# sony/DiffRoll

Measured on AMD Instinct MI355X. Metric: piano-roll frames/sec (200-step sample), higher is better.
Workload: dtype f32

## Files before the change

diffroll_amd/_cabi.py:

```python
from __future__ import annotations

import ctypes as C
import os

_HERE = os.path.dirname(os.path.abspath(__file__))
LIB_PATH = os.environ.get("DR_LIB") or os.path.join(_HERE, "lib", "libdiffroll_amd.so")

DR_ABI_VERSION = 11
DR_OK, DR_EINVAL, DR_ESTATE, DR_EHIP, DR_ENOMEM, DR_ENAME, DR_ETIMEOUT = 0, -1, -2, -3, -4, -5, -6

SAMPLERS = {
    "ddpm_x0": 0,
    "cfdg_ddpm_x0": 1,
    "generation_ddpm_x0": 2,
    "inpainting_ddpm_x0": 3,
    "ddim_x0": 4,
    "cfdg_ddim_x0": 5,
    "ddpm": 6,
    "ddim": 7,
    "ddim2ddpm": 8,
}
COND_SPEC, COND_UNCOND = 0, 1
PRECISIONS = {"f32": 0, "bf16x3": 1, "bf16": 2, "f16": 4}
NORM_MODES = {"imagewise": 0, "framewise": 1}

EXPORTS = [
    "dr_abi_version", "dr_create", "dr_destroy", "dr_last_error", "dr_set_param", "dr_set_tables", "dr_set_frontend_tables",
    "dr_commit", "dr_frontend", "dr_forward", "dr_forward_steps", "dr_step", "dr_sample", "dr_sample_checked", "dr_finish",
    "dr_pending_timeout", "dr_launch_state", "dr_note_runs", "dr_frame_counts", "dr_q_sample", "dr_extract_x0",
    "dr_set_spec_norm", "dr_set_precision", "dr_set_option",
    "dr_comm_unique_id", "dr_comm_create", "dr_comm_destroy", "dr_comm_info", "dr_comm_last_error", "dr_gather",
]
DEBUG_EXPORTS = [
    "dr_debug_stft_power", "dr_debug_bounds", "dr_debug_tenants", "dr_debug_kfd_root", "dr_debug_set_option", "dr_debug_ticks",
    "dr_stack_status", "dr_cold_times", "dr_profile_enable", "dr_profile_read", "dr_profile_read_ex",
    "dr_bench_layer", "dr_bench_pointwise", "dr_debug_launch_counts", "dr_debug_threshold", "dr_debug_rescale", "dr_debug_project",
    "dr_debug_momentum",
]
PUBLIC_OPTIONS = ("blocked_accumulation", "fused_rearm", "fused_stack", "fused_tail", "window_overlap", "window_break", "window_blend", "sampling_steps", "draws", "draw_stride",
                  "guidance_t_min", "guidance_t_max", "solver_order", "start_step", "start_noise", "solver_noise", "x0_clip", "x0_threshold", "cfg_rescale",
                  "cfg_project", "cfg_norm", "cfg_momentum", "guidance_stride")
MODES = {0: "none", 1: "per_phase", 2: "fused_stack", 3: "fused_stack+tail"}


class DrConfig(C.Structure):
    _fields_ = [
        ("abi_version", C.c_int32), ("device", C.c_int32),
        ("residual_channels", C.c_int32), ("residual_layers", C.c_int32),
        ("kernel_size", C.c_int32), ("dilation_base", C.c_int32), ("dilation_bound", C.c_int32),
        ("n_mels", C.c_int32), ("timesteps", C.c_int32), ("sample_rate", C.c_int32),
        ("n_fft", C.c_int32), ("hop_length", C.c_int32),
        ("f_min", C.c_float), ("f_max", C.c_float), ("beta_start", C.c_float), ("beta_end", C.c_float),
# ... 89 lines not shown
    lib.dr_profile_read.restype = C.c_int
    lib.dr_profile_read.argtypes = [vp, C.POINTER(C.c_int64), C.POINTER(C.c_double), C.c_int]
    lib.dr_profile_read_ex.restype = C.c_int
    lib.dr_profile_read_ex.argtypes = [vp, C.POINTER(C.c_int64), C.POINTER(C.c_double), C.POINTER(C.c_double),
                                       C.c_char_p, C.c_size_t, C.c_int]
    lib.dr_set_option.restype = C.c_int
    lib.dr_set_option.argtypes = [vp, C.c_char_p, C.c_int]
    lib.dr_stack_status.restype = C.c_int
    lib.dr_stack_status.argtypes = [vp, C.POINTER(C.c_int32), C.POINTER(C.c_int64), C.POINTER(C.c_int64), C.c_int]
    lib.dr_bench_layer.restype = C.c_int
    lib.dr_bench_layer.argtypes = [vp, C.c_int, C.c_int, C.c_int, C.c_int, C.c_int, vp]
    lib.dr_bench_pointwise.restype = C.c_int
    lib.dr_bench_pointwise.argtypes = [vp, C.c_int, C.c_int, C.c_int, vp]
    lib.dr_debug_ticks.restype = C.c_int
    lib.dr_debug_ticks.argtypes = [vp, C.POINTER(C.c_int64), C.POINTER(C.c_int64)]
    lib.dr_debug_launch_counts.restype = C.c_int
    lib.dr_debug_launch_counts.argtypes = [vp, C.POINTER(C.c_int64)]
    lib.dr_debug_threshold.restype = C.c_int
    lib.dr_debug_threshold.argtypes = [vp, vp, vp, C.c_int, C.c_int, C.c_float, vp, vp]
    lib.dr_debug_rescale.restype = C.c_int
    lib.dr_debug_rescale.argtypes = [vp, vp, vp, C.c_int, C.c_int, C.c_float, vp, vp]
    lib.dr_debug_project.restype = C.c_int
    lib.dr_debug_project.argtypes = [vp, vp, vp, C.c_int, C.c_int, C.c_float, vp, vp]
    lib.dr_debug_momentum.restype = C.c_int
    lib.dr_debug_momentum.argtypes = [vp, vp, vp, vp, vp, C.c_int, C.c_int, C.c_float, vp, vp]
    lib.dr_comm_unique_id.restype = C.c_int
    lib.dr_comm_unique_id.argtypes = [C.c_char_p]
    lib.dr_comm_create.restype = C.c_int
    lib.dr_comm_create.argtypes = [C.POINTER(vp), C.c_char_p, C.c_int, C.c_int, C.c_int]
    lib.dr_comm_destroy.restype = None
# ... 12 lines not shown
```

diffroll_amd/build.py:

```python
from __future__ import annotations

import os
import shutil
import subprocess
import sys

HERE = os.path.dirname(os.path.abspath(__file__))
CSRC = os.path.join(HERE, "csrc")
LIBDIR = os.path.join(HERE, "lib")
LIB = os.path.join(LIBDIR, "libdiffroll_amd.so")
SOURCES = ["gemm.hip", "stack.hip", "tail.hip", "update.hip", "threshold.hip", "rescale.hip", "project.hip", "momentum.hip", "stride.hip", "frontend.hip", "pack.hip", "plan.hip", "abi.hip", "debug_abi.hip", "comm.hip"]
HEADERS = [os.path.join(CSRC, h) for h in ("kernels.h", "chain_tables.h", "device_common.h", "gemm_body.h", "persistent.h", "update_quad.h", "threshold_quad.h", "rescale_quad.h", "project_quad.h", "momentum_quad.h", "stride_quad.h", "group_sums.h", "engine_state.h", "device_buffer.h", "captured_chain.h", "fused_mode.h", "launch_plan.h", "tenants.h", "f16_round.h")] + \
          [os.path.join(os.path.dirname(HERE), "include", h) for h in ("diffroll_amd.h", "diffroll_amd_debug.h")]
FLAGS = ["--offload-arch=gfx950", "-O3", "-std=c++17", "-fPIC", "-Wall", "-Wno-unused-function"]


def _hipcc() -> str:
    for cand in (os.environ.get("HIPCC"), shutil.which("hipcc"), "/opt/rocm/bin/hipcc"):
        if cand and os.path.exists(cand):
            return cand
    raise RuntimeError("hipcc not found (need ROCm with gfx950 support)")


def _stale(target: str, deps) -> bool:
    if not os.path.exists(target):
        return True
    t = os.path.getmtime(target)
# ... 77 lines not shown
```

diffroll_amd/csrc/abi.hip:

```cpp
#include "engine_state.h"
#include "tenants.h"

#include <algorithm>
#include <condition_variable>
#include <mutex>

namespace drh {

thread_local std::string g_create_error;
void release_stager(int dev);
std::atomic<int> g_engines[MAX_DEVICES];

struct FusedSlot {
    std::mutex mu;
    std::condition_variable cv;
    dr_engine* owner = nullptr;
    bool claimed = false;
    hipEvent_t done = nullptr;
};
FusedSlot g_slots[MAX_DEVICES];

bool claim_fused_slot(dr_engine* e, hipStream_t st) {
    FusedSlot& s = g_slots[e->cfg.device];
    std::unique_lock<std::mutex> lk(s.mu);
// ... 406 lines not shown
    if (n == "fused_stack_warm") { put(e, e->opt_stack_warm, value); return DR_OK; }
#ifdef DR_FAULT_HOOK
    if (n == "stack_fault_test") { put(e, e->opt_stack_fault, value); return DR_OK; }
#endif
    if (n == "stack_ticks") { put(e, e->stack_dbg_on, value); return DR_OK; }
    if (n.compare(0, 5, "tune.") == 0) {
        Tuning& t = tuning();
        const std::string f = n.substr(5);
        if (f == "ksplit_blocks") {
            if (put(e, t.ksplit_blocks, value)) tuning_epoch().fetch_add(1);
            return DR_OK;
        }
        std::atomic<int>* field = f == "pack_threads" ? &t.pack_threads : f == "tile" ? &t.tile : f == "pw" ? &t.pw : f == "pw_nw" ? &t.pw_nw
                   : f == "pwk" ? &t.pwk : f == "ksplit_max" ? &t.ksplit_max : f == "one_ks" ? &t.one_ks : f == "stack3" ? &t.stack3
                   : f == "stack_fl" ? &t.stack_fl : f == "tail_t4" ? &t.tail_t4 : f == "xcd_n" ? &t.xcd_n : f == "xcd_model" ? &t.xcd_model
                   : f == "s3_eager" ? &t.s3_eager : f == "debug_chunks" ? &t.debug_chunks : nullptr;
        if (!field) return fail(e, DR_ENAME, "unknown option '%s'", name);
        if (put(e, *field, value)) tuning_epoch().fetch_add(1);
        return DR_OK;
    }
    return fail(e, DR_ENAME, "unknown option '%s'", name);
}

int open_chain_call(dr_engine* e, int sampler, int B, int T, const int* step, int& NB, int& i0, hipStream_t st) {
    int rc = check_ready(e, sampler, B, T);
    if (rc) return rc;
    if (step) {
        const int t = *step;
        if (t < 0 || t >= e->S) return fail(e, DR_EINVAL, "step %d out of range", t);
        if (e->steps.position(t) < 0)
            return fail(e, DR_EINVAL, "step %d is not visited by the respaced chain (option sampling_steps = %d)", t, e->opt.steps);
// ... 530 lines not shown
```

diffroll_amd/csrc/debug_abi.hip:

```cpp
#include "engine_state.h"
#include "tenants.h"

using namespace drh;

extern "C" {

int dr_debug_set_option(dr_engine* e, const char* name, int value) { return drh::set_option(e, name, value, true); }

int dr_debug_threshold(dr_engine* e, const float* d_x0c, const float* d_x0u, int B, int T, float w, float* d_out, void* stream) {
    return drh::debug_threshold(e, d_x0c, d_x0u, B, T, w, d_out, (hipStream_t)stream);
}

int dr_debug_rescale(dr_engine* e, const float* d_x0c, const float* d_x0u, int B, int T, float w, float* d_out, void* stream) {
    return drh::debug_rescale(e, d_x0c, d_x0u, B, T, w, d_out, (hipStream_t)stream);
}

int dr_debug_project(dr_engine* e, const float* d_x0c, const float* d_x0u, int B, int T, float w, float* d_out, void* stream) {
    return drh::debug_project(e, d_x0c, d_x0u, B, T, w, d_out, (hipStream_t)stream);
}

int dr_debug_momentum(dr_engine* e, const float* d_x0c, const float* d_x0u, const float* d_m_prev, float* d_m_next, int B, int T, float w,
                      float* d_out, void* stream) {
    return drh::debug_momentum(e, d_x0c, d_x0u, d_m_prev, d_m_next, B, T, w, d_out, (hipStream_t)stream);
}
// ... 185 lines not shown
    if (!e || !e->dbg_ticks) return fail(e, DR_ESTATE, "no dr_bench_layer launch yet");
    DeviceGuard guard(e->cfg.device);
    long long h[16];
    HIPCHK(e, hipDeviceSynchronize());
    HIPCHK(e, hipMemcpy(h, e->dbg_ticks, sizeof h, hipMemcpyDeviceToHost));
    if (loop_ticks) *loop_ticks = h[0];
    if (block_ticks) *block_ticks = h[1];
    if (tuning().debug_chunks) {
        fprintf(stderr, "[dr] chunk-start ticks since block start:");
        for (int i = 2; i < 16; ++i) fprintf(stderr, " %lld", h[i]);
        fprintf(stderr, "\n");
    }
    return DR_OK;
}

int dr_debug_launch_counts(dr_engine* e, int64_t* out2) {
    if (!e || !out2) return fail(e, DR_EINVAL, "null argument");
    out2[0] = e->inproj_launches;
    out2[1] = e->conv0_launches;
    return DR_OK;
}

}
```

diffroll_amd/csrc/device_common.h:

```cpp
#pragma once
#include "kernels.h"

#include <algorithm>
#include <cstdio>
#include <cstdlib>
#include <type_traits>

namespace dr {

typedef float f32x16 __attribute__((ext_vector_type(16)));
typedef float f32x4 __attribute__((ext_vector_type(4)));
typedef unsigned u32x4 __attribute__((ext_vector_type(4)));

#define DR_DEVINL __device__ __forceinline__

#ifndef DR_FAULT
#define DR_FAULT 0
#endif

#ifdef DR_BOUNDS
static __device__ unsigned long long g_bounds[4];
DR_DEVINL void bounds_fail(unsigned code, long a, long b) {
    if (atomicCAS(&g_bounds[0], 0ull, (unsigned long long)code) == 0ull) { g_bounds[1] = (unsigned long long)a; g_bounds[2] = (unsigned long long)b; }
    atomicAdd(&g_bounds[3], 1ull);
// ... 50 lines not shown
#else
#define DR_CHECK_EXTENTS(a, epi, prec, kernel) do {} while (0)
#define DR_CHECK(cond, code, a, b) do {} while (0)
#define DR_CHECK_LDS(p, lo, hi, code) do {} while (0)
#define DR_BOUNDS_TU(tag)                                                                      \
    hipError_t read_bounds_##tag(unsigned long long*) { return hipErrorNotSupported; }         \
    hipError_t reset_bounds_##tag() { return hipErrorNotSupported; }
#endif
hipError_t read_bounds_gemm(unsigned long long*);  hipError_t reset_bounds_gemm();
hipError_t read_bounds_stack(unsigned long long*); hipError_t reset_bounds_stack();
hipError_t read_bounds_tail(unsigned long long*);  hipError_t reset_bounds_tail();
hipError_t init_stack_kernels();
hipError_t init_tail_kernels();
hipError_t init_frontend_kernels();

struct AF4 { float4 v[4]; };
struct AF6 { uint4 v[6]; };
struct AF2 { uint4 v[2]; };
typedef __bf16 bf16x8 __attribute__((ext_vector_type(8)));
typedef _Float16 f16x8 __attribute__((ext_vector_type(8)));
typedef _Float16 f16x2 __attribute__((ext_vector_type(2)));

template <class... K>
static hipError_t allow_max_lds(K*... kernels) {
    hipError_t e = hipSuccess;
    (void)(((e = hipFuncSetAttribute(reinterpret_cast<const void*>(kernels), hipFuncAttributeMaxDynamicSharedMemorySize, 160 * 1024)) == hipSuccess) && ...);
    return e;
}

DR_DEVINL void f4arr(const float4 v, float (&o)[4]) { o[0] = v.x; o[1] = v.y; o[2] = v.z; o[3] = v.w; }
// ... 151 lines not shown
```

diffroll_amd/csrc/gemm.hip:

```cpp
#include "gemm_body.h"

namespace dr {

Tuning& tuning() { static Tuning t; return t; }
std::atomic<unsigned>& tuning_epoch() { static std::atomic<unsigned> n{0}; return n; }
PlanKnobs plan_knobs() {
    const Tuning& t = tuning();
    PlanKnobs k;
    k.tile = t.tile; k.pw = t.pw; k.pw_nw = t.pw_nw; k.pwk = t.pwk; k.ksplit_max = t.ksplit_max;
    k.ksplit_blocks = t.ksplit_blocks; k.stack3 = t.stack3; k.stack_fl = t.stack_fl;
    k.xcd_n = t.xcd_n; k.xcd_model = t.xcd_model; k.tail_t4 = t.tail_t4; k.one_ks = t.one_ks;
    return k;
}

DR_BOUNDS_TU(gemm)
hipError_t read_bounds(unsigned long long* out4) {
    unsigned long long t[4];
    hipError_t e;
    out4[0] = out4[1] = out4[2] = out4[3] = 0;
    hipError_t (*readers[])(unsigned long long*) = {read_bounds_gemm, read_bounds_stack, read_bounds_tail};
    for (auto rd : readers) {
        if ((e = rd(t)) != hipSuccess) return e;
        if (!out4[0] && t[0]) { out4[0] = t[0]; out4[1] = t[1]; out4[2] = t[2]; }
        out4[3] += t[3];
// ... 228 lines not shown
    return allow_max_lds(&gemm16_kernel<3, 1, EPI_GATE>, &gemm16_kernel<5, 1, EPI_GATE>,
                         &gemm16_kernel<3, 2, EPI_RES_SKIP>, &gemm16_kernel<5, 2, EPI_RES_SKIP>);
}

template <int NI, int KS, int EPI, int PREC>
static hipError_t launch_gemm_t(const GemmArgs& a, hipStream_t s) {
    const int BN = gemm_block_frames(NI);
    const int tps = (a.T + BN - 1) / BN;
    const size_t lds = gemm_lds_bytes(NI, KS, a.taps, a.dil, PREC, EPI);
    if (lds > 160 * 1024) return hipErrorInvalidValue;
    const int NT = a.NB * tps;
    GemmArgs b = a;
    b.ksplit = 1;
    if (a.ws && a.ws_cnt) b.ksplit = plan_ksplit(plan_knobs(), (long)a.MT * NT, a.kchunks / KS, a.kchunks, a.taps, NI, PREC, a.ws_floats, a.ws_cnt_n).ks;
    b.lds_bytes = (int)lds;
    const dim3 grid((unsigned)(a.MT * NT * b.ksplit));
    b.xcd_n = pick_xcd_mapping(a, NT, BN);
    DR_CHECK_EXTENTS(b, EPI, PREC, "gemm_kernel");
    if constexpr (NI == 2 && KS == 1 && EPI == EPI_GATE) {
        if (a.fold128) {
            hipLaunchKernelGGL((gemm_kernel<2, 1, EPI_GATE, PREC, 1>), grid, dim3(512), lds, s, b);
            return hipGetLastError();
        }
    }
    if constexpr (NI == 1 && KS == 1 && EPI == EPI_GATE && PREC == 0) {
        if (a.nofold64 && b.ksplit == 1) {
            hipLaunchKernelGGL((gemm_kernel<1, 1, EPI_GATE, 0, 0>), grid, dim3(512), lds, s, b);
            return hipGetLastError();
        }
    }
// ... 122 lines not shown
```

diffroll_amd/csrc/gemm_body.h:

```cpp
#pragma once
#include "device_common.h"

namespace dr {

DR_DEVINL void residual_quad(const float (&v)[4], const float4 bias, const float4 prev, float (&o)[4]) {
    float bb[4], pv[4];
    f4arr(bias, bb); f4arr(prev, pv);
#pragma unroll
    for (int e = 0; e < 4; ++e) o[e] = div_sqrt2(pv[e] + (v[e] + bb[e]));
}
DR_DEVINL void skip_quad(const float (&v)[4], const float4 bias, const float4 prev, const bool skip_init, float (&o)[4]) {
    float bb[4], pv[4];
    f4arr(bias, bb); f4arr(prev, pv);
#pragma unroll
    for (int e = 0; e < 4; ++e) o[e] = skip_init ? v[e] + bb[e] : (v[e] + bb[e]) + pv[e];
}
DR_DEVINL long cond_row(const GemmArgs& a, const int b) {
    int r = a.c_b0 + b;
    if (a.c_n > 0 && r >= a.c_n) r %= a.c_n;
    return r;
}
DR_DEVINL void gate_quad(const float (&v0)[4], const float (&v1)[4], const float4 bias0, const float4 bias1,
                         const float4 cond0, const float4 cond1, const bool has_c, float (&o)[4]) {
    float b0[4], b1[4], c0[4], c1[4];
// ... 309 lines not shown
            at(F_{}, T_{}, 0);
            int q = 1;
            for (; q + 2 <= per_chunk; q += 2) {
                at(T_{}, F_{}, q);
                at(F_{}, F_{}, q + 1);
            }
            if (q < per_chunk) at(T_{}, F_{}, q);
            else wA = wB;
        }
    } else {
    const __amdgpu_buffer_rsrc_t wrsrc = __builtin_amdgcn_make_buffer_rsrc(
        (void*)(a.Wp + (long)mt * NS * 4096), 0, (unsigned)NS * 16384u, 0x00020000);
    const int wvo = (hi * 128 + wave * 32 + r) * 16;
    auto load_a = [&](int slab) { return load_a4(wrsrc, wvo, slab, NS, 105); };

    AF4 wA = load_a(c0 * KS * a.taps), wB;
    const int cen = (a.taps - 1) >> 1;

    struct BF { float4 v[NW]; };
    BF b0, b1;
    auto xaddr = [&](int chunk, int q) -> const float4* {
        const int j = q / KS, sub = q - j * KS;
        return Xs + (((chunk - c0) & 1) * XP + sub * 8 + hi) * FW + halo + (j - cen) * a.dil + r;
    };
    auto rd = [&](const float4* Xb, int g) -> BF {
        BF o;
#pragma unroll
        for (int ni = 0; ni < NW; ++ni) {
            DR_CHECK_LDS(Xb + g * 2 * FW + ni * 32, xs0, xs1, 106);
            o.v[ni] = Xb[g * 2 * FW + ni * 32];
        }
        return o;
    };
    auto mma4 = [&](auto FIRST, const float4 af, const BF& bf) {
        constexpr bool kFirst = FOLD && decltype(FIRST)::value;
#pragma unroll
        for (int ni = 0; ni < NW; ++ni) acc[ni] = __builtin_amdgcn_mfma_f32_32x32x2f32(af.x, bf.v[ni].x, kFirst ? zero16 : acc[ni], 0, 0, 0);
#pragma unroll
        for (int ni = 0; ni < NW; ++ni) acc[ni] = __builtin_amdgcn_mfma_f32_32x32x2f32(af.y, bf.v[ni].y, acc[ni], 0, 0, 0);
#pragma unroll
        for (int ni = 0; ni < NW; ++ni) acc[ni] = __builtin_amdgcn_mfma_f32_32x32x2f32(af.z, bf.v[ni].z, acc[ni], 0, 0, 0);
#pragma unroll
        for (int ni = 0; ni < NW; ++ni) acc[ni] = __builtin_amdgcn_mfma_f32_32x32x2f32(af.w, bf.v[ni].w, acc[ni], 0, 0, 0);
    };

    const int per_chunk = a.taps * KS;
    auto step = [&](auto ROLE, auto FIRST, int slab, int chunk, int q) {
        constexpr bool kB = decltype(ROLE)::value;
        const float4* Xb = xaddr(chunk, q);
        if constexpr (kB) wA = load_a(min(slab + 1, NS - 1));
        else wB = load_a(min(slab + 1, NS - 1));
        b1 = rd(Xb, 1);
        mma4(FIRST, kB ? wB.v[0] : wA.v[0], b0);
        b0 = rd(Xb, 2);
        mma4(std::false_type{}, kB ? wB.v[1] : wA.v[1], b1);
        b1 = rd(Xb, 3);
        mma4(std::false_type{}, kB ? wB.v[2] : wA.v[2], b0);
        b0 = rd(xaddr(chunk, min(q + 1, per_chunk - 1)), 0);
        mma4(std::false_type{}, kB ? wB.v[3] : wA.v[3], b1);
        sgb<0x100, NW>(); sgb_spread<4, NW>();
        sgb<0x100, NW>(); sgb<0x8, 4 * NW>();
        sgb<0x100, NW>(); sgb<0x8, 4 * NW>();
        sgb<0x100, NW>(); sgb<0x8, 4 * NW>();
    };
    using T_ = std::true_type;
    using F_ = std::false_type;
    constexpr bool AINP = (NI == 2 || NI == 5) && FOLD;
    auto load_ag = [&](int slab, int g) -> float4 {
        DR_CHECK(slab >= 0 && wvo + slab * 16384 + g * 4096 + 16 <= NS * 16384, 112, slab, NS);
        return buffer_load_f4(wrsrc, wvo, slab * 16384 + g * 4096);
    };
    auto stepi = [&](auto FIRST, int slab, int chunk, int q) {
        const float4* Xb = xaddr(chunk, q);
        const int nx = min(slab + 1, NS - 1);
        b1 = rd(Xb, 1);
        mma4(FIRST, wA.v[0], b0);
        wA.v[0] = load_ag(nx, 0);
        b0 = rd(Xb, 2);
        mma4(F_{}, wA.v[1], b1);
        wA.v[1] = load_ag(nx, 1);
        b1 = rd(Xb, 3);
        mma4(F_{}, wA.v[2], b0);
        wA.v[2] = load_ag(nx, 2);
        b0 = rd(xaddr(chunk, min(q + 1, per_chunk - 1)), 0);
        mma4(F_{}, wA.v[3], b1);
        wA.v[3] = load_ag(nx, 3);
        sgb<0x100, NW>(); sgb<0x8, 4 * NW>(); sgb<0x20, 1>();
        sgb<0x100, NW>(); sgb<0x8, 4 * NW>(); sgb<0x20, 1>();
        sgb<0x100, NW>(); sgb<0x8, 4 * NW>(); sgb<0x20, 1>();
        sgb<0x100, NW>(); sgb<0x8, 4 * NW>(); sgb<0x20, 1>();
    };

    for (int chunk = c0; chunk < c1; ++chunk) {
        auto slab_of = [&](int q) {
            const int j = q / KS, sub = q - j * KS;
            return (chunk * KS + sub) * a.taps + j;
        };
        auto at = [&](auto R, auto FIRST, int q) { step(R, FIRST, slab_of(q), chunk, q); };
        __syncthreads();
        if (a.dbg && blockIdx.x == 0 && tid == 0 && chunk < 14) a.dbg[2 + chunk] = clock64() - tick0;
        b0 = rd(xaddr(chunk, 0), 0);
        fold();
        if constexpr (FOLD) __builtin_amdgcn_sched_barrier(0);
        if constexpr (AINP) {
            stepi(T_{}, slab_of(0), chunk, 0);
            int q = 1;
            for (; q + 2 <= per_chunk; q += 2) {
                stepi(F_{}, slab_of(q), chunk, q);
                stepi(F_{}, slab_of(q + 1), chunk, q + 1);
            }
            if (q < per_chunk) stepi(F_{}, slab_of(q), chunk, q);
        } else {
            at(F_{}, T_{}, 0);
            int q = 1;
            for (; q + 2 <= per_chunk; q += 2) {
                at(T_{}, F_{}, q);
                at(F_{}, F_{}, q + 1);
            }
            if (q < per_chunk) at(T_{}, F_{}, q);
            else wA = wB;
        }
    }

    }
    if constexpr (FOLD) {
#pragma unroll
// ... 511 lines not shown
```

diffroll_amd/csrc/kernels.h:

```cpp
#pragma once
#include <hip/hip_runtime.h>
#include <stdint.h>

#include <atomic>

#include "chain_tables.h"
#include "launch_plan.h"

namespace dr {


struct Tuning {
    std::atomic<int> pack_threads{16};
    std::atomic<int> tile{0};
    std::atomic<int> pw{1};
    std::atomic<int> pw_nw{0};
    std::atomic<int> pwk{1};
    std::atomic<int> ksplit_max{16};
    std::atomic<long> ksplit_blocks{0};
    std::atomic<int> one_ks{0};
    std::atomic<int> stack3{1};
    std::atomic<int> stack_fl{0};
    std::atomic<int> tail_t4{0};
    std::atomic<int> xcd_n{-1};
    std::atomic<int> xcd_model{1};
    std::atomic<int> s3_eager{0};
    std::atomic<int> debug_chunks{0};
};
Tuning& tuning();
std::atomic<unsigned>& tuning_epoch();
PlanKnobs plan_knobs();

struct GemmArgs {
    const float* Wp;
    const float* bias;
    const float* bias2;
    const float* X;
    long x_bs, x_ps, x_fs;
    long x_piece;
    int x_planes;
    int x_bmod;
    int NB, T;
// ... 13 lines not shown
    const float* cond;
    long c_bs;
    int c_b0, c_n;
    const float* cond2;
    int n_cond;
    int dual;
    float* skip;
    long s_bs;
    int skip_init;
    float alpha;
    int xcd_n;
    float* ws;
    unsigned* ws_cnt;
    size_t ws_floats, ws_cnt_n;
    int ksplit;
    long long* dbg;
    int lds_bytes;
    int fold128;
    int nofold64;
    int wt_store;
};

hipError_t init_kernels();
hipError_t read_bounds(unsigned long long* out4);
hipError_t reset_bounds();
hipError_t launch_gemm(const GemmArgs& a, int epi, int NI, hipStream_t s, int prec = 0);
hipError_t launch_gemm16(const GemmArgs& a, int epi, int NJ, hipStream_t s);
hipError_t launch_pointwise(const GemmArgs& a, int NW, hipStream_t s);
hipError_t launch_round_bf16(const float* src, float* dst, int NB, int Cp, int T, hipStream_t s);
hipError_t launch_round_f16(const float* src, float* dst, int NB, int Cp, int T, hipStream_t s);
hipError_t launch_pointwise_ksplit(const GemmArgs& a, int NW, hipStream_t s);

struct StackLayer {
    const float *conv_w, *conv_b, *conv_b2;
    const float *cond, *cond2;
    const float *out_w, *out_b;
    int dil, pad_;
};
struct StackArgs {
    float *h, *hd, *g, *skip;
    const float* d2;
    const int* tsel;
    long d2_ts;
    const float* zero;
    int NB, T, Cp, taps, n_cond, L;
    long c_bs;
    int c_b0, c_n;
    int p0, p1;
    int xcd_n;
    int rs_off;
    int lds_bytes;
    int fault;
// ... 128 lines not shown
    float* tmp;
    float* x0;
    const float *skip_w, *skip_b, *outp_w, *outp_b, *zero;
    UpdateArgs u;
    float* x_out;
    const float *in_w, *in_b, *d2_next;
    float *h, *hd;
    const float *conv_w, *conv_b, *conv_b2, *cond, *cond2;
    long c_bs;
    int c_n;
    int taps, dil;
    int fold;
    int t4_ni;
    float* g;
    int lds_bytes;
    long long* dbg;
    unsigned *bar, *pbar, *err, *derr;
    unsigned* ready;
    unsigned epoch;
};
hipError_t launch_tail(const TailArgs& s, hipStream_t st);

hipError_t launch_reflect_pad(const float* wav, float* out, int B, int L, int pad, hipStream_t s);
hipError_t launch_stft_power(const float* wav_pad, const float* win, const float* tw, float* power, int B, int Lp, int TF,
                             int N, int hop, int bins_p, float norm, hipStream_t s);
hipError_t launch_minmax(const float* logmel, float* mm, float* scratch, int B, int planes, int TF, int n_rows, hipStream_t s);
size_t minmax_scratch_floats(int B);
hipError_t launch_minmax_frame(const float* logmel, float* mm, int B, int planes, int TF, int n_rows, hipStream_t s);
hipError_t launch_normalize(const float* logmel, const float* mm, float* specP4, float* spec_plain,
                            int B, int planes_in, int planes_out, int TF, int T, int n_rows,
// ... 12 lines not shown
```

diffroll_amd/csrc/stack.hip:

```cpp
#include "gemm_body.h"
#include "persistent.h"

namespace dr {

DR_BOUNDS_TU(stack)

template <int FL, int FOLDP = 1, int PREC = 0>
__global__ __launch_bounds__(512) void stack_kernel(const StackArgs s_by_value) {
    extern __shared__ __attribute__((aligned(16))) char smem[];
    (void)s_by_value;
    typedef const __attribute__((address_space(4))) StackArgs* KernArgs;
    const KernArgs sp = (KernArgs)__builtin_amdgcn_kernarg_segment_ptr();
    const __attribute__((address_space(4))) StackArgs& s = *sp;
    static_assert(FL == 1 || FL == 2 || (FL == 5 && FOLDP == 1 && PREC == 0), "block flavours");
    constexpr int BN = FL == 5 ? 160 : 64 * FL;
    constexpr int RP = 32;
    constexpr int RWL = (BN + 63) / 64;
    const int wave = __builtin_amdgcn_readfirstlane(threadIdx.x >> 6);
    const int MT = s.Cp >> 6;
    const int MB = MT;
    const int tps = (s.T + BN - 1) / BN;
    const unsigned gsize = (unsigned)(MB * tps);
    int mt, nt, grp, member;
    if (s.xcd_n) {
// ... 84 lines not shown
                const int tps64 = (s.T + 63) >> 6;
                const int b_ = nt / tps, ti = nt % tps;
#pragma unroll 1
                for (int half = 0; half < BN / 64; ++half) {
                    const int t64 = ti * (BN / 64) + half;
                    if (half) {
                        asm volatile("s_waitcnt vmcnt(0)" ::: "memory");
                        __syncthreads();
                    }
                    if (!idle && t64 < tps64) gemm_body<1, 4, EPI_RES_SKIP, PREC, 1>(a, smem, mt, b_ * tps64 + t64, 0);
                }
            }
        } else
        if ((p & 1) == 0) {
            a.Wp = ly.conv_w; a.bias = ly.conv_b; a.bias2 = ly.conv_b2;
            a.X = s.hd; a.taps = s.taps; a.dil = ly.dil;
            a.cond = ly.cond; a.cond2 = ly.cond2; a.c_bs = s.c_bs; a.c_b0 = s.c_b0; a.c_n = s.c_n; a.n_cond = s.n_cond;
            a.Y = s.g;
            if (s.dbg && p + 2 >= s.p1) a.dbg = s.dbg + 64;
            gemm_body<FL, 1, EPI_GATE, 0, 1, FOLDP>(a, smem, mt, nt, 0);
            if (wave == 4) __builtin_amdgcn_fence(__ATOMIC_ACQUIRE, "agent");
            if (wave >= 4 && s.warm) {
                const int be = nt / tps;
                if (be < s.n_cond)
                    l2_touch(ly.cond + cond_row(a, be) * s.c_bs + (long)mt * 32 * s.T * 4, (unsigned)(32 * s.T * 16), wave - 4, 4);
                l2_touch(ly.out_w + (long)mt * (s.Cp >> 5) * 4096, (unsigned)((s.Cp >> 5) * 16384), wave - 4, 4);
            }
        } else {
            a.Wp = ly.out_w; a.bias = ly.out_b;
            a.X = s.g; a.taps = 1; a.dil = 1;
            a.Y = s.h;
// ... 70 lines not shown
    else if (b.fold128) hipLaunchKernelGGL((stack_kernel<2, 1, PREC>), grid, dim3(512), lds, st, b);
    else hipLaunchKernelGGL((stack_kernel<2, 0, PREC>), grid, dim3(512), lds, st, b);
    return hipGetLastError();
}

hipError_t launch_stack(const StackArgs& s, int FL, int max_dil, hipStream_t st, int prec) {
    if (FL != 1 && FL != 2 && FL != 5) return hipErrorInvalidValue;
    if (prec && ((s.Cp & 127) || FL == 5)) return hipErrorInvalidValue;
    if (s.L < 1 || s.L > DR_STACK_MAX_LAYERS || s.p0 < 0 || s.p1 > 2 * s.L || s.p0 >= s.p1 || (s.Cp & 63)) return hipErrorInvalidValue;
    const int BN = stack_tile_frames(FL), MT = s.Cp >> 6, gsize = stack_group_blocks(FL, s.Cp, s.T);
    const size_t lds = prec ? stack3_lds_bytes(FL, s.taps, max_dil, prec) : stack_lds_bytes(FL, s.taps, max_dil);
    if (lds > 160 * 1024) return hipErrorInvalidValue;
    StackArgs b = s;
    b.rs_off = (int)(lds - 16 - (size_t)32 * BN * 16);
    b.lds_bytes = (int)lds;
    const int NBp = xcd_padded_groups(s.NB, gsize, &b.xcd_n);
#ifdef DR_BOUNDS
    for (int l = 0; l < s.L; ++l) {
        GemmArgs g{};
        g.MT = MT; g.NB = s.NB; g.T = s.T; g.taps = s.taps; g.kchunks = s.Cp >> 5; g.y_rows = s.Cp;
        g.x_bs = g.y_bs = g.y2_bs = g.s_bs = (long)s.Cp * s.T; g.x_ps = g.y_ps = (long)s.T * 4; g.x_fs = g.y_fs = 4; g.x_planes = s.Cp >> 2;
        g.Wp = s.layer[l].conv_w; g.bias = s.layer[l].conv_b; g.bias2 = s.layer[l].conv_b2; g.X = s.hd; g.Y = s.g;
        g.cond = s.layer[l].cond; g.cond2 = s.layer[l].cond2; g.c_bs = s.c_bs; g.c_b0 = s.c_b0; g.c_n = s.c_n; g.n_cond = s.n_cond;
        check_gemm_extents(g, EPI_GATE, 0, "stack_kernel (conv phase)");
        g.taps = 1; g.Wp = s.layer[l].out_w; g.bias = s.layer[l].out_b; g.X = s.g; g.Y = s.h; g.Y2 = s.hd; g.skip = s.skip;
        check_gemm_extents(g, EPI_RES_SKIP, 0, "stack_kernel (1x1 phase)");
    }
    host_extent(s.bar, (size_t)4 * 512 * 4, "group counters", "stack_kernel");
    host_extent(s.xid, (size_t)1024 * 4, "tag words", "stack_kernel");
#endif
// ... 22 lines not shown
```

diffroll_amd/csrc/tail.hip:

```cpp
#include "gemm_body.h"
#include "persistent.h"
#include "update_quad.h"

namespace dr {

DR_BOUNDS_TU(tail)

__global__ __launch_bounds__(512) void tail_kernel(const TailArgs s) {
    extern __shared__ __attribute__((aligned(16))) char smem[];
    float4* XT = reinterpret_cast<float4*>(smem);
    const int wave = __builtin_amdgcn_readfirstlane(threadIdx.x >> 6);
    const int lane = threadIdx.x & 63;
    const int MT = s.Cp >> 6;
    const int tps = (s.T + s.BN - 1) / s.BN;
    const unsigned gsize = (unsigned)(MT * tps);
    int grp, member;
    if (s.xcd_n) {
        const int xcd = blockIdx.x & 7, idx = blockIdx.x >> 3;
        member = idx % (int)gsize;
        grp = (idx / (int)gsize) * 8 + xcd;
    } else {
        member = blockIdx.x % (int)gsize;
        grp = blockIdx.x / (int)gsize;
    }
// ... 119 lines not shown
            }
        }
    }
    mark();
    if (s.dual_next > 0 && s.conv_w) {
        if (paired) group_barrier<false>(pctr, 2u * (2u * gsize + DR_FAULT_EXTRA(s)), s.err, s.derr);
        else group_barrier<false>(ctr, 3u * (gsize + DR_FAULT_EXTRA(s)), s.err, s.derr);
        mark();
        GemmArgs a{};
        a.d2 = s.zero; a.wt_store = 0;
        a.lds_bytes = s.lds_bytes;
        a.MT = MT; a.NB = s.dual_next; a.T = s.T; a.alpha = 1.f; a.ksplit = 1;
        a.x_bs = act_bs; a.x_ps = (long)s.T * 4; a.x_fs = 4; a.x_planes = P; a.kchunks = s.Cp >> 5;
        a.y_bs = act_bs; a.y_ps = (long)s.T * 4; a.y_fs = 4; a.y_rows = s.Cp;
        a.Wp = s.conv_w; a.bias = s.conv_b; a.bias2 = s.conv_b2;
        a.X = s.hd; a.taps = s.taps; a.dil = s.dil;
        a.cond = s.cond; a.cond2 = s.cond2; a.c_bs = s.c_bs; a.c_n = s.c_n; a.n_cond = s.dual_next;
        a.dual = s.dual_next;
        a.Y = s.g;
        const int bn4 = s.t4_ni == 3 ? 96 : 64;
        const int tps4 = (s.T + bn4 - 1) / bn4;
        const int n4 = MT * tps4;
        for (int it = pair_half * (int)gsize + member; it < n4; it += (paired ? 2 : 1) * (int)gsize) {
            asm volatile("s_waitcnt vmcnt(0)" ::: "memory");
            __syncthreads();
            if (s.t4_ni == 3) gemm_body<3, 1, EPI_GATE, 0, 1, 1>(a, smem, it % MT, pair_i * tps4 + it / MT, 0);
            else if (s.fold) gemm_body<1, 1, EPI_GATE, 0, 1, 1>(a, smem, it % MT, pair_i * tps4 + it / MT, 0);
            else gemm_body<1, 1, EPI_GATE, 0, 1, 0>(a, smem, it % MT, pair_i * tps4 + it / MT, 0);
        }
    }
    if (s.dbg && blockIdx.x == 0 && threadIdx.x == 0) s.dbg[7] = clock64();
// ... 20 lines not shown
    if (s.dual_next < 0 || (s.dual_next > 0 && (s.dual_next != s.u_B || s.u_B != (s.dual > 0 ? s.dual : s.NB)))) return hipErrorInvalidValue;
    if (!s.x_out || s.x_out == s.u.x) return hipErrorInvalidValue;
    if (win_H(s.u) > 0 && (!s.ready || s.u_B > STACK_GROUPS || 2 * win_H(s.u) < s.T || win_H(s.u) >= s.T)) return hipErrorInvalidValue;
    if (s.u.win_tab && win_H(s.u) <= 0) return hipErrorInvalidValue;
    const int tps = (s.T + s.BN - 1) / s.BN, MT = s.Cp >> 6;
    TailArgs b = s;
    const int NBp = xcd_padded_groups(s.NB, MT * tps, &b.xcd_n);
    size_t lds = 24 * 32 * 16;
    if (s.conv_w) {
        if (s.dual_next <= 0 || !s.in_w || (s.taps & 1) == 0) return hipErrorInvalidValue;
        b.t4_ni = tail_t4_width(s.fold, s.t4_ni, s.dual > 0, MT, s.T, s.BN);
        lds = std::max(lds, gemm_lds_bytes(b.t4_ni, 1, s.taps, s.dil, 0, EPI_GATE));
        if (lds > 160 * 1024) return hipErrorInvalidValue;
    }
    b.lds_bytes = (int)lds;
    hipLaunchKernelGGL(tail_kernel, dim3((unsigned)(MT * tps * NBp)), dim3(512), lds, st, b);
    return hipGetLastError();
}

hipError_t init_tail_kernels() {
    return allow_max_lds(&tail_kernel);
}

}
```

include/diffroll_amd_debug.h:

```cpp
#ifndef DIFFROLL_AMD_DEBUG_H
#define DIFFROLL_AMD_DEBUG_H

#include "diffroll_amd.h"

#ifdef __cplusplus
extern "C" {
#endif

int dr_debug_stft_power(dr_engine* e, const float* d_wav, int B, int L, float* d_power_out, void* stream);

int dr_debug_bounds(int64_t* out4, int reset);

int dr_debug_tenants(const char* kfd_root, int pci_domain, int pci_bus, int pci_device, int64_t* out4);
int dr_debug_kfd_root(const char* kfd_root);

int dr_debug_set_option(dr_engine* e, const char* name, int value);

int dr_stack_status(dr_engine* e, int32_t* timed_out, int64_t* launches, int64_t* ticks, int n_ticks);

int dr_cold_times(dr_engine* e, double* out5);

int dr_profile_enable(dr_engine* e, int on);
int dr_profile_read(dr_engine* e, int64_t* launches, double* total_ms, int reset);
int dr_profile_read_ex(dr_engine* e, int64_t* launches, double* total_ms, double* total_flops, char* name,
                       size_t name_len, int reset);

int dr_bench_layer(dr_engine* e, int layer, int NB, int T, int t, int n_cond, void* stream);
int dr_bench_pointwise(dr_engine* e, int layer, int NB, int T, void* stream);
int dr_debug_ticks(dr_engine* e, int64_t* loop_ticks, int64_t* block_ticks);

int dr_debug_launch_counts(dr_engine* e, int64_t* out2);

int dr_debug_threshold(dr_engine* e, const float* d_x0c, const float* d_x0u, int B, int T, float w, float* d_out, void* stream);

int dr_debug_rescale(dr_engine* e, const float* d_x0c, const float* d_x0u, int B, int T, float w, float* d_out, void* stream);

int dr_debug_project(dr_engine* e, const float* d_x0c, const float* d_x0u, int B, int T, float w, float* d_out, void* stream);

int dr_debug_momentum(dr_engine* e, const float* d_x0c, const float* d_x0u, const float* d_m_prev, float* d_m_next, int B, int T, float w,
                      float* d_out, void* stream);

#ifdef __cplusplus
}
#endif
#endif
```

Before: 2256.

## Skip MFMA tiles that read only zero padding in dilated conv GEMM

Adds a pad-skip path to the gated conv GEMM body. When the first or last tap of a dilated convolution maps a whole 32-column tile entirely outside [0,T), that tile's MFMAs and LDS reads are dropped, using compile-time tile ranges and a runtime choice among four specialised variants. The aim is to avoid MFMA work on padding in edge tiles of dilated layers. The cost is more template instantiations (code size, register pressure) and extra first-accumulate handling. The path is on by default through the pad_skip tuning option.

```diff
diff --git a/diffroll_amd/_cabi.py b/diffroll_amd/_cabi.py
--- a/diffroll_amd/_cabi.py
+++ b/diffroll_amd/_cabi.py
@@ -35,7 +35,7 @@
     "dr_debug_stft_power", "dr_debug_bounds", "dr_debug_tenants", "dr_debug_kfd_root", "dr_debug_set_option", "dr_debug_ticks",
     "dr_stack_status", "dr_cold_times", "dr_profile_enable", "dr_profile_read", "dr_profile_read_ex",
     "dr_bench_layer", "dr_bench_pointwise", "dr_debug_launch_counts", "dr_debug_threshold", "dr_debug_rescale", "dr_debug_project",
-    "dr_debug_momentum",
+    "dr_debug_momentum", "dr_debug_pad_mfmas",
 ]
 PUBLIC_OPTIONS = ("blocked_accumulation", "fused_rearm", "fused_stack", "fused_tail", "window_overlap", "window_break", "window_blend", "sampling_steps", "draws", "draw_stride",
                   "guidance_t_min", "guidance_t_max", "solver_order", "start_step", "start_noise", "solver_noise", "x0_clip", "x0_threshold", "cfg_rescale",
@@ -155,6 +155,8 @@
     lib.dr_bench_pointwise.argtypes = [vp, C.c_int, C.c_int, C.c_int, vp]
     lib.dr_debug_ticks.restype = C.c_int
     lib.dr_debug_ticks.argtypes = [vp, C.POINTER(C.c_int64), C.POINTER(C.c_int64)]
+    lib.dr_debug_pad_mfmas.restype = C.c_int64
+    lib.dr_debug_pad_mfmas.argtypes = [C.c_int] * 7
     lib.dr_debug_launch_counts.restype = C.c_int
     lib.dr_debug_launch_counts.argtypes = [vp, C.POINTER(C.c_int64)]
     lib.dr_debug_threshold.restype = C.c_int
diff --git a/diffroll_amd/build.py b/diffroll_amd/build.py
--- a/diffroll_amd/build.py
+++ b/diffroll_amd/build.py
@@ -10,7 +10,7 @@
 LIBDIR = os.path.join(HERE, "lib")
 LIB = os.path.join(LIBDIR, "libdiffroll_amd.so")
 SOURCES = ["gemm.hip", "stack.hip", "tail.hip", "update.hip", "threshold.hip", "rescale.hip", "project.hip", "momentum.hip", "stride.hip", "frontend.hip", "pack.hip", "plan.hip", "abi.hip", "debug_abi.hip", "comm.hip"]
-HEADERS = [os.path.join(CSRC, h) for h in ("kernels.h", "chain_tables.h", "device_common.h", "gemm_body.h", "persistent.h", "update_quad.h", "threshold_quad.h", "rescale_quad.h", "project_quad.h", "momentum_quad.h", "stride_quad.h", "group_sums.h", "engine_state.h", "device_buffer.h", "captured_chain.h", "fused_mode.h", "launch_plan.h", "tenants.h", "f16_round.h")] + \
+HEADERS = [os.path.join(CSRC, h) for h in ("kernels.h", "chain_tables.h", "device_common.h", "gemm_body.h", "persistent.h", "update_quad.h", "threshold_quad.h", "rescale_quad.h", "project_quad.h", "momentum_quad.h", "stride_quad.h", "group_sums.h", "engine_state.h", "device_buffer.h", "captured_chain.h", "fused_mode.h", "launch_plan.h", "pad_tiles.h", "tenants.h", "f16_round.h")] + \
           [os.path.join(os.path.dirname(HERE), "include", h) for h in ("diffroll_amd.h", "diffroll_amd_debug.h")]
 FLAGS = ["--offload-arch=gfx950", "-O3", "-std=c++17", "-fPIC", "-Wall", "-Wno-unused-function"]
 
diff --git a/diffroll_amd/csrc/abi.hip b/diffroll_amd/csrc/abi.hip
--- a/diffroll_amd/csrc/abi.hip
+++ b/diffroll_amd/csrc/abi.hip
@@ -444,7 +444,7 @@
         std::atomic<int>* field = f == "pack_threads" ? &t.pack_threads : f == "tile" ? &t.tile : f == "pw" ? &t.pw : f == "pw_nw" ? &t.pw_nw
                    : f == "pwk" ? &t.pwk : f == "ksplit_max" ? &t.ksplit_max : f == "one_ks" ? &t.one_ks : f == "stack3" ? &t.stack3
                    : f == "stack_fl" ? &t.stack_fl : f == "tail_t4" ? &t.tail_t4 : f == "xcd_n" ? &t.xcd_n : f == "xcd_model" ? &t.xcd_model
-                   : f == "s3_eager" ? &t.s3_eager : f == "debug_chunks" ? &t.debug_chunks : nullptr;
+                   : f == "s3_eager" ? &t.s3_eager : f == "debug_chunks" ? &t.debug_chunks : f == "pad_skip" ? &t.pad_skip : nullptr;
         if (!field) return fail(e, DR_ENAME, "unknown option '%s'", name);
         if (put(e, *field, value)) tuning_epoch().fetch_add(1);
         return DR_OK;
diff --git a/diffroll_amd/csrc/debug_abi.hip b/diffroll_amd/csrc/debug_abi.hip
--- a/diffroll_amd/csrc/debug_abi.hip
+++ b/diffroll_amd/csrc/debug_abi.hip
@@ -1,4 +1,5 @@
 #include "engine_state.h"
+#include "pad_tiles.h"
 #include "tenants.h"
 
 using namespace drh;
@@ -223,6 +224,11 @@
     return DR_OK;
 }
 
+int64_t dr_debug_pad_mfmas(int T, int t0, int taps, int dil, int NW, int kchunks, int pad_skip) {
+    if (T < 1 || t0 < 0 || taps < 1 || dil < 1 || NW < 1 || kchunks < 1) return -1;
+    return dr::pad_wave_mfmas(T, t0, taps, dil, NW, kchunks, pad_skip);
+}
+
 int dr_debug_launch_counts(dr_engine* e, int64_t* out2) {
     if (!e || !out2) return fail(e, DR_EINVAL, "null argument");
     out2[0] = e->inproj_launches;
diff --git a/diffroll_amd/csrc/device_common.h b/diffroll_amd/csrc/device_common.h
--- a/diffroll_amd/csrc/device_common.h
+++ b/diffroll_amd/csrc/device_common.h
@@ -88,6 +88,8 @@
 hipError_t init_tail_kernels();
 hipError_t init_frontend_kernels();
 
+template <int LO, int HI>
+struct Tiles { static constexpr int lo = LO, hi = HI; };
 struct AF4 { float4 v[4]; };
 struct AF6 { uint4 v[6]; };
 struct AF2 { uint4 v[2]; };
diff --git a/diffroll_amd/csrc/gemm.hip b/diffroll_amd/csrc/gemm.hip
--- a/diffroll_amd/csrc/gemm.hip
+++ b/diffroll_amd/csrc/gemm.hip
@@ -266,6 +266,7 @@
     b.ksplit = 1;
     if (a.ws && a.ws_cnt) b.ksplit = plan_ksplit(plan_knobs(), (long)a.MT * NT, a.kchunks / KS, a.kchunks, a.taps, NI, PREC, a.ws_floats, a.ws_cnt_n).ks;
     b.lds_bytes = (int)lds;
+    b.pad_skip = tuning().pad_skip;
     const dim3 grid((unsigned)(a.MT * NT * b.ksplit));
     b.xcd_n = pick_xcd_mapping(a, NT, BN);
     DR_CHECK_EXTENTS(b, EPI, PREC, "gemm_kernel");
diff --git a/diffroll_amd/csrc/gemm_body.h b/diffroll_amd/csrc/gemm_body.h
--- a/diffroll_amd/csrc/gemm_body.h
+++ b/diffroll_amd/csrc/gemm_body.h
@@ -1,5 +1,6 @@
 #pragma once
 #include "device_common.h"
+#include "pad_tiles.h"
 
 namespace dr {
 
@@ -347,7 +348,9 @@
     const int wvo = (hi * 128 + wave * 32 + r) * 16;
     auto load_a = [&](int slab) { return load_a4(wrsrc, wvo, slab, NS, 105); };
 
-    AF4 wA = load_a(c0 * KS * a.taps), wB;
+    constexpr bool PADSKIP = EPI == EPI_GATE && KS == 1 && (NI == 1 || NI == 2);
+    AF4 wA, wB;
+    if constexpr (!PADSKIP) wA = load_a(c0 * KS * a.taps);
     const int cen = (a.taps - 1) >> 1;
 
     struct BF { float4 v[NW]; };
@@ -356,45 +359,49 @@
         const int j = q / KS, sub = q - j * KS;
         return Xs + (((chunk - c0) & 1) * XP + sub * 8 + hi) * FW + halo + (j - cen) * a.dil + r;
     };
-    auto rd = [&](const float4* Xb, int g) -> BF {
+    using AllTiles = Tiles<0, NW>;
+    auto rd = [&](const float4* Xb, int g, auto TILES) -> BF {
         BF o;
 #pragma unroll
-        for (int ni = 0; ni < NW; ++ni) {
+        for (int ni = decltype(TILES)::lo; ni < decltype(TILES)::hi; ++ni) {
             DR_CHECK_LDS(Xb + g * 2 * FW + ni * 32, xs0, xs1, 106);
             o.v[ni] = Xb[g * 2 * FW + ni * 32];
         }
         return o;
     };
-    auto mma4 = [&](auto FIRST, const float4 af, const BF& bf) {
-        constexpr bool kFirst = FOLD && decltype(FIRST)::value;
-#pragma unroll
-        for (int ni = 0; ni < NW; ++ni) acc[ni] = __builtin_amdgcn_mfma_f32_32x32x2f32(af.x, bf.v[ni].x, kFirst ? zero16 : acc[ni], 0, 0, 0);
-#pragma unroll
-        for (int ni = 0; ni < NW; ++ni) acc[ni] = __builtin_amdgcn_mfma_f32_32x32x2f32(af.y, bf.v[ni].y, acc[ni], 0, 0, 0);
-#pragma unroll
-        for (int ni = 0; ni < NW; ++ni) acc[ni] = __builtin_amdgcn_mfma_f32_32x32x2f32(af.z, bf.v[ni].z, acc[ni], 0, 0, 0);
-#pragma unroll
-        for (int ni = 0; ni < NW; ++ni) acc[ni] = __builtin_amdgcn_mfma_f32_32x32x2f32(af.w, bf.v[ni].w, acc[ni], 0, 0, 0);
+    auto mma4 = [&](auto FIRST, auto TILES, const float4 af, const BF& bf) {
+        constexpr int kFirst = FOLD ? (int)decltype(FIRST)::value : 0;
+        constexpr int LO = decltype(TILES)::lo, HI = decltype(TILES)::hi;
+#pragma unroll
+        for (int ni = LO; ni < HI; ++ni)
+            acc[ni] = __builtin_amdgcn_mfma_f32_32x32x2f32(af.x, bf.v[ni].x, (kFirst == 1 || (kFirst == 2 && ni == 0)) ? zero16 : acc[ni], 0, 0, 0);
+#pragma unroll
+        for (int ni = LO; ni < HI; ++ni) acc[ni] = __builtin_amdgcn_mfma_f32_32x32x2f32(af.y, bf.v[ni].y, acc[ni], 0, 0, 0);
+#pragma unroll
+        for (int ni = LO; ni < HI; ++ni) acc[ni] = __builtin_amdgcn_mfma_f32_32x32x2f32(af.z, bf.v[ni].z, acc[ni], 0, 0, 0);
+#pragma unroll
+        for (int ni = LO; ni < HI; ++ni) acc[ni] = __builtin_amdgcn_mfma_f32_32x32x2f32(af.w, bf.v[ni].w, acc[ni], 0, 0, 0);
     };
 
     const int per_chunk = a.taps * KS;
-    auto step = [&](auto ROLE, auto FIRST, int slab, int chunk, int q) {
+    auto step = [&](auto ROLE, auto FIRST, auto TILES, int slab, int chunk, int q) {
         constexpr bool kB = decltype(ROLE)::value;
+        constexpr int NR = decltype(TILES)::hi - decltype(TILES)::lo;
         const float4* Xb = xaddr(chunk, q);
         if constexpr (kB) wA = load_a(min(slab + 1, NS - 1));
         else wB = load_a(min(slab + 1, NS - 1));
-        b1 = rd(Xb, 1);
-        mma4(FIRST, kB ? wB.v[0] : wA.v[0], b0);
-        b0 = rd(Xb, 2);
-        mma4(std::false_type{}, kB ? wB.v[1] : wA.v[1], b1);
-        b1 = rd(Xb, 3);
-        mma4(std::false_type{}, kB ? wB.v[2] : wA.v[2], b0);
-        b0 = rd(xaddr(chunk, min(q + 1, per_chunk - 1)), 0);
-        mma4(std::false_type{}, kB ? wB.v[3] : wA.v[3], b1);
-        sgb<0x100, NW>(); sgb_spread<4, NW>();
-        sgb<0x100, NW>(); sgb<0x8, 4 * NW>();
-        sgb<0x100, NW>(); sgb<0x8, 4 * NW>();
-        sgb<0x100, NW>(); sgb<0x8, 4 * NW>();
+        b1 = rd(Xb, 1, TILES);
+        mma4(FIRST, TILES, kB ? wB.v[0] : wA.v[0], b0);
+        b0 = rd(Xb, 2, TILES);
+        mma4(std::false_type{}, TILES, kB ? wB.v[1] : wA.v[1], b1);
+        b1 = rd(Xb, 3, TILES);
+        mma4(std::false_type{}, TILES, kB ? wB.v[2] : wA.v[2], b0);
+        b0 = rd(xaddr(chunk, min(q + 1, per_chunk - 1)), 0, AllTiles{});
+        mma4(std::false_type{}, TILES, kB ? wB.v[3] : wA.v[3], b1);
+        sgb<0x100, NR>(); sgb_spread<4, NR>();
+        sgb<0x100, NR>(); sgb<0x8, 4 * NR>();
+        sgb<0x100, NR>(); sgb<0x8, 4 * NR>();
+        sgb<0x100, NW>(); sgb<0x8, 4 * NR>();
     };
     using T_ = std::true_type;
     using F_ = std::false_type;
@@ -403,46 +410,90 @@
         DR_CHECK(slab >= 0 && wvo + slab * 16384 + g * 4096 + 16 <= NS * 16384, 112, slab, NS);
         return buffer_load_f4(wrsrc, wvo, slab * 16384 + g * 4096);
     };
-    auto stepi = [&](auto FIRST, int slab, int chunk, int q) {
+    auto stepi = [&](auto FIRST, auto TILES, int slab, int chunk, int q) {
+        constexpr int NR = decltype(TILES)::hi - decltype(TILES)::lo;
         const float4* Xb = xaddr(chunk, q);
         const int nx = min(slab + 1, NS - 1);
-        b1 = rd(Xb, 1);
-        mma4(FIRST, wA.v[0], b0);
+        b1 = rd(Xb, 1, TILES);
+        mma4(FIRST, TILES, wA.v[0], b0);
         wA.v[0] = load_ag(nx, 0);
-        b0 = rd(Xb, 2);
-        mma4(F_{}, wA.v[1], b1);
+        b0 = rd(Xb, 2, TILES);
+        mma4(F_{}, TILES, wA.v[1], b1);
         wA.v[1] = load_ag(nx, 1);
-        b1 = rd(Xb, 3);
-        mma4(F_{}, wA.v[2], b0);
+        b1 = rd(Xb, 3, TILES);
+        mma4(F_{}, TILES, wA.v[2], b0);
         wA.v[2] = load_ag(nx, 2);
-        b0 = rd(xaddr(chunk, min(q + 1, per_chunk - 1)), 0);
-        mma4(F_{}, wA.v[3], b1);
+        b0 = rd(xaddr(chunk, min(q + 1, per_chunk - 1)), 0, AllTiles{});
+        mma4(F_{}, TILES, wA.v[3], b1);
         wA.v[3] = load_ag(nx, 3);
-        sgb<0x100, NW>(); sgb<0x8, 4 * NW>(); sgb<0x20, 1>();
-        sgb<0x100, NW>(); sgb<0x8, 4 * NW>(); sgb<0x20, 1>();
-        sgb<0x100, NW>(); sgb<0x8, 4 * NW>(); sgb<0x20, 1>();
-        sgb<0x100, NW>(); sgb<0x8, 4 * NW>(); sgb<0x20, 1>();
-    };
-
+        sgb<0x100, NR>(); sgb<0x8, 4 * NR>(); sgb<0x20, 1>();
+        sgb<0x100, NR>(); sgb<0x8, 4 * NR>(); sgb<0x20, 1>();
+        sgb<0x100, NR>(); sgb<0x8, 4 * NR>(); sgb<0x20, 1>();
+        sgb<0x100, NW>(); sgb<0x8, 4 * NR>(); sgb<0x20, 1>();
+    };
+
+    if constexpr (PADSKIP) {
+        auto chunks = [&](auto DF, auto DL) {
+            using Tiles0 = std::conditional_t<decltype(DF)::value, Tiles<1, NW>, AllTiles>;
+            using TilesL = std::conditional_t<decltype(DL)::value, Tiles<0, NW - 1>, AllTiles>;
+            using First1 = std::integral_constant<int, decltype(DF)::value ? 2 : 0>;
+            wA = load_a(c0 * KS * a.taps);
+            for (int chunk = c0; chunk < c1; ++chunk) {
+                auto one = [&](auto R, auto FIRST, auto TILES, int q) {
+                    const int slab = chunk * a.taps + q;
+                    if constexpr (AINP) stepi(FIRST, TILES, slab, chunk, q);
+                    else step(R, FIRST, TILES, slab, chunk, q);
+                };
+                __syncthreads();
+                if (a.dbg && blockIdx.x == 0 && tid == 0 && chunk < 14) a.dbg[2 + chunk] = clock64() - tick0;
+                b0 = rd(xaddr(chunk, 0), 0, AllTiles{});
+                fold();
+                if constexpr (FOLD) __builtin_amdgcn_sched_barrier(0);
+                one(F_{}, T_{}, Tiles0{}, 0);
+                if (per_chunk > 1) one(T_{}, First1{}, AllTiles{}, 1);
+                int q = 2;
+                for (; q + 2 <= per_chunk; q += 2) {
+                    one(F_{}, F_{}, AllTiles{}, q);
+                    one(T_{}, F_{}, AllTiles{}, q + 1);
+                }
+                if (q < per_chunk) one(F_{}, F_{}, TilesL{}, q);
+                if constexpr (!AINP) {
+                    if (per_chunk & 1) wA = wB;
+                }
+            }
+        };
+        bool drop_first = false, drop_last = false;
+        if (a.pad_skip) {
+            drop_first = pad_step_form(a.T, t0, a.taps, a.dil, 0, NW) == PAD_DROP_FIRST;
+            drop_last = pad_step_form(a.T, t0, a.taps, a.dil, a.taps - 1, NW) == PAD_DROP_LAST;
+        }
+        if (drop_first) {
+            if (drop_last) chunks(T_{}, T_{});
+            else chunks(T_{}, F_{});
+        } else {
+            if (drop_last) chunks(F_{}, T_{});
+            else chunks(F_{}, F_{});
+        }
+    } else
     for (int chunk = c0; chunk < c1; ++chunk) {
         auto slab_of = [&](int q) {
             const int j = q / KS, sub = q - j * KS;
             return (chunk * KS + sub) * a.taps + j;
         };
-        auto at = [&](auto R, auto FIRST, int q) { step(R, FIRST, slab_of(q), chunk, q); };
+        auto at = [&](auto R, auto FIRST, int q) { step(R, FIRST, AllTiles{}, slab_of(q), chunk, q); };
         __syncthreads();
         if (a.dbg && blockIdx.x == 0 && tid == 0 && chunk < 14) a.dbg[2 + chunk] = clock64() - tick0;
-        b0 = rd(xaddr(chunk, 0), 0);
+        b0 = rd(xaddr(chunk, 0), 0, AllTiles{});
         fold();
         if constexpr (FOLD) __builtin_amdgcn_sched_barrier(0);
         if constexpr (AINP) {
-            stepi(T_{}, slab_of(0), chunk, 0);
+            stepi(T_{}, AllTiles{}, slab_of(0), chunk, 0);
             int q = 1;
             for (; q + 2 <= per_chunk; q += 2) {
-                stepi(F_{}, slab_of(q), chunk, q);
-                stepi(F_{}, slab_of(q + 1), chunk, q + 1);
-            }
-            if (q < per_chunk) stepi(F_{}, slab_of(q), chunk, q);
+                stepi(F_{}, AllTiles{}, slab_of(q), chunk, q);
+                stepi(F_{}, AllTiles{}, slab_of(q + 1), chunk, q + 1);
+            }
+            if (q < per_chunk) stepi(F_{}, AllTiles{}, slab_of(q), chunk, q);
         } else {
             at(F_{}, T_{}, 0);
             int q = 1;
diff --git a/diffroll_amd/csrc/kernels.h b/diffroll_amd/csrc/kernels.h
--- a/diffroll_amd/csrc/kernels.h
+++ b/diffroll_amd/csrc/kernels.h
@@ -26,6 +26,7 @@
     std::atomic<int> xcd_model{1};
     std::atomic<int> s3_eager{0};
     std::atomic<int> debug_chunks{0};
+    std::atomic<int> pad_skip{1};
 };
 Tuning& tuning();
 std::atomic<unsigned>& tuning_epoch();
@@ -69,6 +70,7 @@
     unsigned* ws_cnt;
     size_t ws_floats, ws_cnt_n;
     int ksplit;
+    int pad_skip;
     long long* dbg;
     int lds_bytes;
     int fold128;
@@ -90,7 +92,8 @@
     const float *conv_w, *conv_b, *conv_b2;
     const float *cond, *cond2;
     const float *out_w, *out_b;
-    int dil, pad_;
+    int dil;
+    int pad_skip;
 };
 struct StackArgs {
     float *h, *hd, *g, *skip;
@@ -249,6 +252,7 @@
     int t4_ni;
     float* g;
     int lds_bytes;
+    int pad_skip;
     long long* dbg;
     unsigned *bar, *pbar, *err, *derr;
     unsigned* ready;
diff --git a/diffroll_amd/csrc/pad_tiles.h b/diffroll_amd/csrc/pad_tiles.h
--- /dev/null
+++ b/diffroll_amd/csrc/pad_tiles.h
@@ -0,0 +1,40 @@
+#pragma once
+
+#if defined(__HIPCC__) || defined(__CUDACC__)
+#define DR_PAD_HD __host__ __device__ inline
+#else
+#define DR_PAD_HD inline
+#endif
+
+namespace dr {
+
+DR_PAD_HD bool pad_tile_dead(int T, int t0, int taps, int dil, int tap, int tile) {
+    const int first = t0 + 32 * tile + (tap - (taps - 1) / 2) * dil;
+    return first + 32 <= 0 || first >= T;
+}
+DR_PAD_HD int pad_tiles_lead(int T, int t0, int taps, int dil, int tap, int NW) {
+    int n = 0;
+    while (n < NW && pad_tile_dead(T, t0, taps, dil, tap, n)) ++n;
+    return n;
+}
+DR_PAD_HD int pad_tiles_trail(int T, int t0, int taps, int dil, int tap, int NW) {
+    int n = 0;
+    while (n < NW && pad_tile_dead(T, t0, taps, dil, tap, NW - 1 - n)) ++n;
+    return n;
+}
+
+enum PadStep : int { PAD_ALL = 0, PAD_DROP_FIRST = 1, PAD_DROP_LAST = 2 };
+DR_PAD_HD int pad_step_form(int T, int t0, int taps, int dil, int tap, int NW) {
+    if (taps < 3 || !(taps & 1)) return PAD_ALL;
+    if (tap == 0 && pad_tile_dead(T, t0, taps, dil, 0, 0)) return PAD_DROP_FIRST;
+    if (tap == taps - 1 && pad_tile_dead(T, t0, taps, dil, tap, NW - 1)) return PAD_DROP_LAST;
+    return PAD_ALL;
+}
+DR_PAD_HD long pad_wave_mfmas(int T, int t0, int taps, int dil, int NW, int kchunks, int pad_skip) {
+    int tiles = 0;
+    for (int tap = 0; tap < taps; ++tap)
+        tiles += NW - ((pad_skip && pad_step_form(T, t0, taps, dil, tap, NW) != PAD_ALL) ? 1 : 0);
+    return 16L * tiles * kchunks;
+}
+
+}
diff --git a/diffroll_amd/csrc/stack.hip b/diffroll_amd/csrc/stack.hip
--- a/diffroll_amd/csrc/stack.hip
+++ b/diffroll_amd/csrc/stack.hip
@@ -122,7 +122,7 @@
         } else
         if ((p & 1) == 0) {
             a.Wp = ly.conv_w; a.bias = ly.conv_b; a.bias2 = ly.conv_b2;
-            a.X = s.hd; a.taps = s.taps; a.dil = ly.dil;
+            a.X = s.hd; a.taps = s.taps; a.dil = ly.dil; a.pad_skip = ly.pad_skip;
             a.cond = ly.cond; a.cond2 = ly.cond2; a.c_bs = s.c_bs; a.c_b0 = s.c_b0; a.c_n = s.c_n; a.n_cond = s.n_cond;
             a.Y = s.g;
             if (s.dbg && p + 2 >= s.p1) a.dbg = s.dbg + 64;
@@ -223,6 +223,7 @@
     StackArgs b = s;
     b.rs_off = (int)(lds - 16 - (size_t)32 * BN * 16);
     b.lds_bytes = (int)lds;
+    for (int l = 0; l < s.L; ++l) b.layer[l].pad_skip = tuning().pad_skip;
     const int NBp = xcd_padded_groups(s.NB, gsize, &b.xcd_n);
 #ifdef DR_BOUNDS
     for (int l = 0; l < s.L; ++l) {
diff --git a/diffroll_amd/csrc/tail.hip b/diffroll_amd/csrc/tail.hip
--- a/diffroll_amd/csrc/tail.hip
+++ b/diffroll_amd/csrc/tail.hip
@@ -157,7 +157,7 @@
         a.x_bs = act_bs; a.x_ps = (long)s.T * 4; a.x_fs = 4; a.x_planes = P; a.kchunks = s.Cp >> 5;
         a.y_bs = act_bs; a.y_ps = (long)s.T * 4; a.y_fs = 4; a.y_rows = s.Cp;
         a.Wp = s.conv_w; a.bias = s.conv_b; a.bias2 = s.conv_b2;
-        a.X = s.hd; a.taps = s.taps; a.dil = s.dil;
+        a.X = s.hd; a.taps = s.taps; a.dil = s.dil; a.pad_skip = s.pad_skip;
         a.cond = s.cond; a.cond2 = s.cond2; a.c_bs = s.c_bs; a.c_n = s.c_n; a.n_cond = s.dual_next;
         a.dual = s.dual_next;
         a.Y = s.g;
@@ -208,6 +208,7 @@
         if (lds > 160 * 1024) return hipErrorInvalidValue;
     }
     b.lds_bytes = (int)lds;
+    b.pad_skip = tuning().pad_skip;
     hipLaunchKernelGGL(tail_kernel, dim3((unsigned)(MT * tps * NBp)), dim3(512), lds, st, b);
     return hipGetLastError();
 }
diff --git a/include/diffroll_amd_debug.h b/include/diffroll_amd_debug.h
--- a/include/diffroll_amd_debug.h
+++ b/include/diffroll_amd_debug.h
@@ -31,6 +31,8 @@
 
 int dr_debug_launch_counts(dr_engine* e, int64_t* out2);
 
+int64_t dr_debug_pad_mfmas(int T, int t0, int taps, int dil, int NW, int kchunks, int pad_skip);
+
 int dr_debug_threshold(dr_engine* e, const float* d_x0c, const float* d_x0u, int B, int T, float w, float* d_out, void* stream);
 
 int dr_debug_rescale(dr_engine* e, const float* d_x0c, const float* d_x0u, int B, int T, float w, float* d_out, void* stream);
```

New measurement: 2274, median of 6. About the same (+0.8%).
